# AHartmaier/pyLabFEA

Measured on AMD Instinct MI355X. Metric: integration-point updates/sec (wall-clock per load step in ms_per_step), higher is better.
Workload: dtype f64

## Files before the change

include/plfx.h:

```cpp
#ifndef PLFX_H
#define PLFX_H

#include <stddef.h>
#include <stdint.h>

#ifdef __cplusplus
extern "C" {
#endif

typedef struct plfx_ctx plfx_ctx;

enum {
    PLFX_ELASTIC = 0,
    PLFX_HILL6 = 1,
    PLFX_PRINC3 = 2,
    PLFX_SVC6 = 3,
    PLFX_TRESCA = 4,
    PLFX_BARLAT = 5,
    PLFX_SVC3 = 6,
    PLFX_SVC_WH = 7,
    PLFX_SVC6_COLS = 8
};

enum {
// ... 90 lines not shown
int plfx_set_precond(plfx_ctx *ctx, int kind, double omega, int nu);
int plfx_precond_info(plfx_ctx *ctx, int *kind_in_use, int *levels);
int plfx_precond_apply(plfx_ctx *ctx, const double *r, double *z);
int plfx_precond_bench(plfx_ctx *ctx, int reps, double *us_per_cycle, double *us_coarse);
int plfx_solve_fallbacks(plfx_ctx *ctx, int64_t *count);
int plfx_indefinite_info(plfx_ctx *ctx, int64_t *solves, int64_t *by_minres_surrogate, int64_t *by_gmres,
                         int64_t *surrogates_built, int64_t *elements_shifted);
int plfx_set_operator(plfx_ctx *ctx, int kind);
int plfx_matvec(plfx_ctx *ctx, const double *x, double *y);
int plfx_operator_info(plfx_ctx *ctx, int *matrix_free, int *levels_matrix_free);
int plfx_reuse_info(plfx_ctx *ctx, int *assemblies, int *bc_applications, int *solves);
int plfx_predict_info(plfx_ctx *ctx, int64_t *applied, int64_t *skipped, int64_t *rejected);
int plfx_sweep_info(plfx_ctx *ctx, int64_t *sweeps, int64_t *tangents_rewritten);
int plfx_sweep_launch_info(plfx_ctx *ctx, int64_t *heavy_skipped, int64_t *heavy_recovered);
int plfx_bc_info(plfx_ctx *ctx, int64_t *rhs_rows_only, int64_t *dinv_kept, int64_t *dinv_refreshed, int64_t *du_early);
int plfx_dead_store_info(plfx_ctx *ctx, int64_t *armed_sweeps, int64_t *tangents_rewritten_in_armed_sweeps,
                         int64_t *test_only_starts, int64_t *test_only_retries);
enum {
    PLFX_PLANE_ON = 0,
    PLFX_PLANE_NEVER_ON = 1,
    PLFX_PLANE_SWITCH = 2,
    PLFX_PLANE_SHARDED = 3,
    PLFX_PLANE_MATERIALS = 4,
    PLFX_PLANE_STATE_SET = 5,
    PLFX_PLANE_TANGENT_SET = 6
};
int plfx_plane_info(plfx_ctx *ctx, int *mode_on, int64_t *plane_sweeps, int64_t *plane_updates, int *switched_off_by);
enum {
    PLFX_MG_TAIL_NONE = 0,
    PLFX_MG_TAIL_GENERIC = 1,
// ... 133 lines not shown
```

pylabfea_amd/_lib.py:

```python
import ctypes as C
import os

import numpy as np

_HERE = os.path.dirname(os.path.abspath(__file__))
LIB_PATH = os.environ.get('PLFX_LIB', os.path.join(_HERE, 'libplfx.so'))

ELASTIC, HILL6, PRINC3, SVC6, TRESCA, BARLAT, SVC3, SVC_WH, SVC6_COLS = 0, 1, 2, 3, 4, 5, 6, 7, 8

ST_SIG, ST_EPS, ST_EPL, ST_RES_SIG, ST_RES_DEPL, ST_ELSTIFF, ST_U, ST_F, ST_DU, ST_FYN, ST_MAXSTEPS, ST_KHARD = range(12)

FIELD_NAMES = ('strain1', 'strain2', 'strain12', 'stress1', 'stress2', 'stress12', 'plastic1', 'plastic2', 'plastic12',
               'seq', 'seqJ2', 'peeq', 'etot', 'ux', 'uy')
FIELD_ID = {n: i for i, n in enumerate(FIELD_NAMES)}

T_SWEEP, T_SPMV, T_CGUPD, T_ASSEMBLE, T_VCYCLE, T_SMOOTH, T_SWEEP_HEAVY, T_COMM = range(8)


class PlfxError(RuntimeError):
    pass


class CMaterial(C.Structure):
    _fields_ = [('kind', C.c_int32), ('sdim', C.c_int32), ('CV', C.c_double * 36),
# ... 17 lines not shown
    'plfx_precond_info', 'plfx_set_operator', 'plfx_operator_info', 'plfx_gen_structured', 'plfx_reuse_info', 'plfx_timing_select', 'plfx_finish_fetch', 'plfx_sweep_info', 'plfx_matvec', 'plfx_set_bc_plan', 'plfx_apply_bc_plan',
    'plfx_set_finish_set', 'plfx_finish_step', 'plfx_scf_all', 'plfx_comm_info', 'plfx_comm_init_callback',
    'plfx_set_bc_sources',
    'plfx_load_step', 'plfx_set_strip', 'plfx_strip_info', 'plfx_allreduce_host',
    'plfx_response_batch_kh', 'plfx_fgrad_batch_wh', 'plfx_timing_sample', 'plfx_solve_fallbacks', 'plfx_comm_selftest',
    'plfx_indefinite_info', 'plfx_pattern_selftest', 'plfx_precond_bench', 'plfx_set_wh_mode', 'plfx_wh_info', 'plfx_wh_carry', 'plfx_set_mesh_structured',
    'plfx_svc_info', 'plfx_fgrad_seq_batch', 'plfx_precond_apply', 'plfx_predict_info',
    'plfx_set_response_maxit', 'plfx_sig_princ_host', 'plfx_eig3_host',
    'plfx_svc_fit_batch', 'plfx_svc_decision_batch', 'plfx_svc_fit_wide', 'plfx_hessian_batch',
    'plfx_svr_fit_batch', 'plfx_svr_predict_multi', 'plfx_set_svr_flow', 'plfx_svr_flow_info',
    'plfx_sweep_launch_info', 'plfx_element_fields', 'plfx_bc_info', 'plfx_yield_scale',
    'plfx_committee_yf', 'plfx_committee_info',
    'plfx_tex_svc_set', 'plfx_tex_svc_yf', 'plfx_tex_svc_yield_scale', 'plfx_tex_svc_info',
    'plfx_tex_svc_fgrad', 'plfx_tex_svc_full_yf', 'plfx_tex_svc_response', 'plfx_tex_svc_flow_info',
    'plfx_flow_curve', 'plfx_flow_info',
    'plfx_dead_store_info', 'plfx_plane_info',
    'plfx_set_svc_cols', 'plfx_mg_info',
    'plfx_set_svc_textures', 'plfx_set_element_textures', 'plfx_response_batch_tid', 'plfx_full_yf_batch_tid',
    'plfx_svc_textures_info',
]

_lib = None


def load():
    global _lib
    if _lib is not None:
        return _lib
    if not os.path.exists(LIB_PATH):
        raise PlfxError('libplfx.so not found at %s - build it first (__graft_entry__.build()); '
                        'pylabfea_amd has no CPU fallback' % LIB_PATH)
# ... 609 lines not shown
    def sweep_info(self):
        a, b = C.c_int64(), C.c_int64()
        self._chk(self.lib.plfx_sweep_info(self.h, C.byref(a), C.byref(b)))
        return a.value, b.value

    def sweep_launch_info(self):
        a, b = C.c_int64(), C.c_int64()
        self._chk(self.lib.plfx_sweep_launch_info(self.h, C.byref(a), C.byref(b)))
        return a.value, b.value

    def bc_info(self):
        a, b, r, d = C.c_int64(), C.c_int64(), C.c_int64(), C.c_int64()
        self._chk(self.lib.plfx_bc_info(self.h, C.byref(a), C.byref(b), C.byref(r), C.byref(d)))
        return a.value, b.value, r.value, d.value

    def dead_store_info(self):
        a, b, r, d = C.c_int64(), C.c_int64(), C.c_int64(), C.c_int64()
        self._chk(self.lib.plfx_dead_store_info(self.h, C.byref(a), C.byref(b), C.byref(r), C.byref(d)))
        return a.value, b.value, r.value, d.value

    PLANE_OFF_REASONS = ('on', 'no state reset yet', 'switch', 'sharded', 'materials', 'state_set', 'tangent set')

    def plane_info(self):
        on, a, b, why = C.c_int(), C.c_int64(), C.c_int64(), C.c_int()
        self._chk(self.lib.plfx_plane_info(self.h, C.byref(on), C.byref(a), C.byref(b), C.byref(why)))
        return bool(on.value), a.value, b.value, why.value

    MG_TAIL_KERNELS = ('none', 'tail', 'tail_lds', 'tail_mf', 'tail_mf_ragged')
    MG_COARSE_SOLVERS = ('dense', 'cheby', 'pcg')

# ... 310 lines not shown
```

pylabfea_amd/csrc/plfx.hip:

```cpp
#include "../../include/plfx.h"
#include "plfx_kernels.hpp"
#include "plfx_mg.hpp"
#include "plfx_tex.hpp"
#include "plfx_texflow.hpp"
#include "plfx_flow.hpp"

#include <dlfcn.h>
#include <algorithm>
#include <chrono>
#include <thread>
#include <cmath>
#include <cstdarg>
#include <cstdio>
#include <cstring>
#include <map>
#include <mutex>
#include <string>
#include <type_traits>
#include <vector>

using namespace plfx;

#define PLFX_VERSION "0.1.0-r1"

// ... 190 lines not shown
    std::vector<int32_t> bc_idx;
    bool bc_valid = false;
    double *stage = nullptr;
    size_t stage_cap = 0;
    hipEvent_t stage_ev[2] = {nullptr, nullptr};
    bool stage_busy[2] = {false, false};
    int stage_flip = 0;
    int32_t *bc_idx_dev = nullptr;
    size_t bc_idx_cap = 0;
    int32_t *bc_rows = nullptr;
    int bc_nrows = 0;
    double *kw = nullptr;
    bool bc_rows_on = true;
    bool rhs_rows_ok = false, dinv_ok = false;
    long long n_rhs_rows = 0, n_dinv_kept = 0, n_dinv_refreshed = 0, n_du_early = 0;
    int last_heavy = -1;
    long long n_heavy_skipped = 0, n_heavy_recovered = 0;
    bool x_is_du = false;
    double *pred_x = nullptr, *pred_d = nullptr;
    bool pred_valid = false;
    bool predict = true;
    bool mg_pending = false, mg_pending_same = true;
    long long n_mg_setup = 0, n_mg_setup_skipped = 0;
    bool spec_arm = false, spec_setup = false, spec_kdu = false, spec_was_clean = false;
    bool dead_stores = true, test_starts = true, dead_arm = false, res_partial = false;
    long long n_dead_sweeps = 0, n_dead_tangents = 0, n_test_starts = 0, n_test_retries = 0;
    bool plane_switch = true, plane_mats_ok = false, plane_cols = false;
    int plane_off_by = PLFX_PLANE_NEVER_ON;
    long long n_plane_sweeps = 0, n_plane_updates = 0;
    bool first_test_hint[2] = {false, false};
// ... 574 lines not shown
    dfree(c->f);
    dfree(c->du);
    dfree(c->rhs);
    dfree(c->dinv);
    dfree(c->diag);
    dfree(c->is_presc);
    dfree(c->dup);
    dfree(c->wv);
    dfree(c->fext);
    dfree(c->x);
    dfree(c->r);
    dfree(c->z);
    dfree(c->q);
    dfree(c->pred_x);
    dfree(c->pred_d);
    c->pred_valid = false;
    for (auto &b : c->gm_blk) dfree(b);
    c->gm_blk.clear();
    c->gm_m = 0;
    dfree(c->gm_part);
    dfree(c->gm_part2);
    dfree(c->gm_red);
    dfree(c->gm_coef);
    dfree(c->p[0]);
    dfree(c->p[1]);
    for (auto &L : c->mg) {
        if (!L.owned) continue;
        dfree(L.col);
        dfree(L.contrib);
        dfree(L.cls0);
        dfree(L.val);
// ... 18 lines not shown
    c->val_valid = false;
    c->mg_tail = -1;
    c->gx = c->gy = 0;
    c->assembled = c->bc_set = false;
    c->M_dirty = true;
    c->x_is_du = false;
    c->bc_valid = false;
    c->bc_idx.clear();
    c->plan.valid = false;
    dfree(c->fin_idx);
    dfree(c->fin_dev);
    c->fin_n = 0;
    dfree(c->kw);
    dfree(c->bc_rows);
    c->bc_nrows = 0;
    c->rhs_rows_ok = c->dinv_ok = false;
    dfree(c->tex_ids);
    c->htex_ids.clear();
    c->tex_ids_ok = false;
}

void free_tex_field(plfx_ctx *c, int k)
{
    TexFieldDev &f = c->tex_field[k];
    if (f.coef) hipFree((void *)f.coef);
    if (f.sabs) hipFree((void *)f.sabs);
    f = TexFieldDev();
    c->tex_field_mask &= ~(1u << k);
    c->tex_field_rows[k] = 0;
    c->tex_field_launches[k] = 0;
    c->tex_ids_ok = false;
// ... 254 lines not shown
    KOp o;
    o.rx = rx;
    o.ry = ry;
    o.nnode = nnode;
    o.nslot = nslot;
    o.col = col;
    o.val = val;
    o.nxn = nx + 1;
    o.nyn = ny + 1;
    o.nel = nel;
    o.M = M;
    o.tab = c->dtab;
    return o;
}

int assemble_fine_val(plfx_ctx *c)
{
    hipLaunchKernelGGL(k_assemble, dim3(grid_for(c->nnode), c->nslot), dim3(BLOCK), 0, c->stream,
                       c->dcls, c->ncls, c->nnode, c->nslot, c->nq, c->nel_total, c->dcontrib, c->dcls_all,
                       (matfree(c) && c->assembled) ? c->Mop : c->Mel, c->dcol, c->dval, c->diag,
                       (matfree(c) && c->assembled) ? 1 : 0);
    HIPCHK(c, hipGetLastError());
    c->dinv_ok = false;
    c->val_valid = true;
    return 0;
}

static bool level_plain(const plfx_ctx::MgLevel &L) { return !(L.nx & 1) && !(L.ny & 1) && L.rx == 1. && L.ry == 1.; }

static bool level_from_generators(const plfx_ctx *c, int l)
{
    return matfree(c) && (c->mg[l].matfree || (tail_mf(c) && l < (int)c->mg.size() - 1));
// ... 241 lines not shown
    c->mg_graph = nullptr;
    auto &S = c->strip;
    if (S.x_down) hipGraphExecDestroy(S.x_down);
    if (S.x_up) hipGraphExecDestroy(S.x_up);
    if (S.g_down) hipGraphDestroy(S.g_down);
    if (S.g_up) hipGraphDestroy(S.g_up);
    S.x_down = S.x_up = nullptr;
    S.g_down = S.g_up = nullptr;
}

int mg_assemble(plfx_ctx *c);
int mg_update_dinv(plfx_ctx *c, bool same_set);
bool mg_lazy(const plfx_ctx *c) { return c->predict && matfree(c) && !c->strip.on && !comm_active(c); }
int mg_ensure(plfx_ctx *c)
{
    if (!c->mg_pending) return 0;
    c->mg_pending = false;
    c->n_mg_setup++;
    int rc = mg_assemble(c);
    if (rc) return rc;
    return mg_update_dinv(c, c->mg_pending_same);
}

int mg_vcycle_head(plfx_ctx *c)
{
    if (c->strip_jacobi) return 0;
    const int nl = (int)c->mg.size();
    const int lt = (c->mg_tail > 0) ? c->mg_tail : nl - 1;
    if (lt >= 1) return mg_down_level(c, 0);
    return 0;
}

int mg_vcycle_rest(plfx_ctx *c, double *rz_part, bool *wrote)
{
// ... 180 lines not shown
    HIPCHK(c, hipStreamCreateWithFlags(&c->stream, hipStreamNonBlocking));
    if (const char *e2 = getenv("PLFX_MATFREE")) c->want_matfree = atoi(e2) ? 1 : 0;
    if (const char *e3 = getenv("PLFX_SVC_WAVE")) c->want_svc_wave = atoi(e3) ? 1 : 0;
    if (const char *e4 = getenv("PLFX_COLL_TIMEOUT")) c->coll_timeout_s = atof(e4);
    if (const char *e4 = getenv("PLFX_MG_GRAPH")) c->want_mg_graph = atoi(e4) ? 1 : 0;
    if (const char *e8 = getenv("PLFX_REUSE")) c->reuse = atoi(e8) != 0;
    if (const char *e9 = getenv("PLFX_BC_ROWS")) c->bc_rows_on = atoi(e9) != 0;
    if (const char *e10 = getenv("PLFX_DEAD_STORES")) {
        const int v = atoi(e10);
        c->dead_stores = v == 1 || v == 2;
        c->test_starts = v == 1 || v == 3;
    }
    if (!c->reuse) c->dead_stores = c->test_starts = false;
    if (const char *e11 = getenv("PLFX_PLANE_COLS")) c->plane_switch = atoi(e11) != 0;
    if (!c->reuse) c->plane_switch = false;
    if (const char *e9 = getenv("PLFX_PREDICT")) c->predict = atoi(e9) != 0;
    {
        const char *e5 = getenv("PLFX_MAILBOX");
        if (!e5 || atoi(e5)) {
            if (hipHostMalloc((void **)&c->mbox, sizeof(CgMbox), hipHostMallocMapped | hipHostMallocCoherent) == hipSuccess)
                memset(c->mbox, 0, sizeof(CgMbox));
            else
                c->mbox = nullptr;
            c->mb_cap = 1 << 16;
            if (c->mbox && hipHostMalloc((void **)&c->mb_buf, (size_t)8 * c->mb_cap,
                                         hipHostMallocMapped | hipHostMallocCoherent) != hipSuccess) {
                c->mb_buf = nullptr;
                c->mb_cap = 0;
            }
        }
// ... 1939 lines not shown
    k->grid_nodes = grid_xcd(k->nnode);
    k->op = make_op(k, k->nnode, 0, nullptr, nullptr, k->gx, k->gy, k->nel_total, k->Mop);
    rc = build_hierarchy(k, k->gx, k->gy, c->hcls[0]);
    if (rc || !mg_active(k)) {
        if (!rc) rc = fail(c, PLFX_ERR_UNSUPPORTED, "the global coarse grid %d x %d has no usable hierarchy", k->gx, k->gy);
        else c->err = k->err;
        strip_free(c);
        return rc;
    }
    S.on = true;
    c->grid_nodes = MAXPART;
    c->assembled = false, c->M_dirty = true;
    c->bc_set = false;
    c->bc_valid = false;
    c->rhs_rows_ok = c->dinv_ok = false;
    c->x_is_du = false;
    c->memo.valid = false;
    return PLFX_OK;
}

int plfx_strip_info(plfx_ctx *c, int *active, int *halo, int *coarse_level, int *coarse_levels, int64_t *halo_refreshes,
                    int64_t *coarse_gathers, int64_t *partial_allreduces, int64_t *generator_exchanges)
{
    if (!c) return PLFX_ERR_ARG;
    const auto &S = c->strip;
    if (active) *active = S.on ? 1 : 0;
    if (halo) *halo = S.W;
    if (coarse_level) *coarse_level = S.Ld;
    if (coarse_levels) *coarse_levels = S.child ? (int)S.child->mg.size() : 0;
    if (halo_refreshes) *halo_refreshes = S.n_halo;
// ... 46 lines not shown
int plfx_sweep_info(plfx_ctx *c, int64_t *sweeps, int64_t *tangents_rewritten)
{
    if (!c) return PLFX_ERR_ARG;
    if (sweeps) *sweeps = c->n_sweeps;
    if (tangents_rewritten) *tangents_rewritten = c->n_tangents_rewritten;
    return PLFX_OK;
}

int plfx_bc_info(plfx_ctx *c, int64_t *rhs_rows_only, int64_t *dinv_kept, int64_t *dinv_refreshed, int64_t *du_early)
{
    if (!c) return PLFX_ERR_ARG;
    if (rhs_rows_only) *rhs_rows_only = c->n_rhs_rows;
    if (dinv_kept) *dinv_kept = c->n_dinv_kept;
    if (dinv_refreshed) *dinv_refreshed = c->n_dinv_refreshed;
    if (du_early) *du_early = c->n_du_early;
    return PLFX_OK;
}

int plfx_dead_store_info(plfx_ctx *c, int64_t *armed_sweeps, int64_t *tangents_rewritten_in_armed_sweeps, int64_t *test_only_starts,
                         int64_t *test_only_retries)
{
    if (!c) return PLFX_ERR_ARG;
    if (armed_sweeps) *armed_sweeps = c->n_dead_sweeps;
    if (tangents_rewritten_in_armed_sweeps) *tangents_rewritten_in_armed_sweeps = c->n_dead_tangents;
    if (test_only_starts) *test_only_starts = c->n_test_starts;
    if (test_only_retries) *test_only_retries = c->n_test_retries;
    return PLFX_OK;
}

int plfx_plane_info(plfx_ctx *c, int *mode_on, int64_t *plane_sweeps, int64_t *plane_updates, int *switched_off_by)
// ... 332 lines not shown
        c->kh_out_valid = false;
    }
    hipLaunchKernelGGL(k_init_tangent, dim3((c->nel + BLOCK - 1) / BLOCK), dim3(BLOCK), 0, c->stream,
                       c->dmat, c->dcls, c->nel, c->dcls_id, tan_store(c), c->Mel + c->e0, c->nel_total);
    if (c->sharded)
        hipLaunchKernelGGL(k_init_M_all, dim3((c->nel_total + BLOCK - 1) / BLOCK), dim3(BLOCK), 0, c->stream,
                           c->dmat, c->dcls, c->nel_total, c->dcls_all, c->Mel);
    HIPCHK(c, hipGetLastError());
    c->plane_off_by = !c->plane_switch ? PLFX_PLANE_SWITCH : (c->sharded || c->strip.on || comm_active(c)) ? PLFX_PLANE_SHARDED :
                      !c->plane_mats_ok ? PLFX_PLANE_MATERIALS : PLFX_PLANE_ON;
    c->plane_cols = c->plane_off_by == PLFX_PLANE_ON;
    if (c->plane_cols) HIPCHK(c, hipMemsetAsync(c->elfac + 4 * ne, 0, 16 * ne, c->stream));
    c->assembled = false, c->M_dirty = true;
    c->x_is_du = false;
    c->rhs_rows_ok = c->dinv_ok = false;
    c->res_is_sig = c->res_fresh = c->eps_stale = c->res_partial = false;
    c->last_heavy = -1;
    return PLFX_OK;
}

static int ensure_eps(plfx_ctx *c)
{
    if (!c->eps_stale) return 0;
    hipLaunchKernelGGL(k_eps_from_u, dim3(grid_for(c->nel, MAXPART)), dim3(BLOCK), 0, c->stream, c->dmat, c->nmat, c->dcls, c->ncls,
                       c->nel, c->e0, c->dconn, c->dcls_id, (const double2 *)c->u, c->eps);
    HIPCHK(c, hipGetLastError());
    c->eps_stale = false;
    return 0;
}

// ... 107 lines not shown

int plfx_state_set(plfx_ctx *c, int which, const double *in)
{
    if (!c || !c->sig) return c ? fail(c, PLFX_ERR_STATE, "set_mesh first") : PLFX_ERR_STATE;
    if (!in) return fail(c, PLFX_ERR_ARG, "null input");
    if (which == 10) return fail(c, PLFX_ERR_ARG, "max_steps is read-only");
    double *p;
    size_t comps, n;
    bool soa;
    int rc = (which == 0 || which == 3) ? split_res_sig(c) : 0;
    if (rc) return rc;
    rc = state_ptr(c, which, &p, &comps, &n, &soa);
    if (rc) return rc;
    if (!soa) {
        c->x_is_du = false;
        HIPCHK(c, hipMemcpyAsync(p, in, 8 * n, hipMemcpyHostToDevice, c->stream));
        HIPCHK(c, stream_sync(c));
        return PLFX_OK;
    }
    std::vector<double> t(comps * n);
    if (comps == 6) {
        for (size_t e = 0; e < n; e++)
            for (int k = 0; k < 6; k++) t[(size_t)k * n + e] = in[6 * e + k];
    } else {
        for (size_t e = 0; e < n; e++)
            for (int i = 0; i < 6; i++)
                for (int j = i; j < 6; j++) t[(size_t)sym_idx(i, j) * n + e] = in[36 * e + 6 * i + j];
    }
    if (c->plane_cols && (which == 0 || which == 2 || which == 3 || which == 4)) {
        const double *c34 = t.data() + 3 * n;
// ... 123 lines not shown
    rowptr[2 * nn] = (int32_t)pos;
    return PLFX_OK;
}

namespace {
int apply_bc_impl(plfx_ctx *c, int n, const int32_t *idx, const double *du_presc, const double *w, const double *fext,
                  const int32_t *seg4, const BcSegVals *segv)
{
    const size_t nd = c->ndof;
    int rc = ensure_tmp(c, std::max(n, 1));
    if (rc) return rc;
    const bool same_set = c->bc_valid && (int)c->bc_idx.size() == n &&
                          (n == 0 || memcmp(c->bc_idx.data(), idx, (size_t)4 * n) == 0);
    if (!same_set) {
        c->x_is_du = false;
        HIPCHK(c, hipMemsetAsync(c->is_presc, 0, 8 * nd, c->stream));
        HIPCHK(c, hipMemsetAsync(c->dup, 0, 8 * nd, c->stream));
        HIPCHK(c, hipMemsetAsync(c->wv, 0, 8 * nd, c->stream));
        c->bc_idx.assign(idx, idx + n);
        if ((size_t)n > c->bc_idx_cap) {
            dfree(c->bc_idx_dev);
            if ((rc = dalloc(c, &c->bc_idx_dev, (size_t)n))) return rc;
            c->bc_idx_cap = n;
        }
        if (n > 0) {
            HIPCHK(c, hipMemcpyAsync(c->bc_idx_dev, c->bc_idx.data(), (size_t)4 * n, hipMemcpyHostToDevice, c->stream));
        }
        {
            std::vector<char> mark(c->nnode, 0);
            const int nn = c->nnode;
// ... 68 lines not shown
    {
        if (matfree(c) && c->op.colr)
            hipLaunchKernelGGL(HIP_KERNEL_NAME(k_spmv_rows<2>), dim3((c->bc_nrows + BLOCK - 1) / BLOCK), dim3(BLOCK), 0,
                               c->stream, c->bc_nrows, c->bc_rows, c->op, (const double2 *)c->wv, (double2 *)c->kw, rm, rr);
        else if (matfree(c))
            hipLaunchKernelGGL(HIP_KERNEL_NAME(k_spmv_rows<1>), dim3((c->bc_nrows + BLOCK - 1) / BLOCK), dim3(BLOCK), 0,
                               c->stream, c->bc_nrows, c->bc_rows, c->op, (const double2 *)c->wv, (double2 *)c->kw, rm, rr);
        else
            hipLaunchKernelGGL(HIP_KERNEL_NAME(k_spmv_rows<0>), dim3((c->bc_nrows + BLOCK - 1) / BLOCK), dim3(BLOCK), 0,
                               c->stream, c->bc_nrows, c->bc_rows, c->op, (const double2 *)c->wv, (double2 *)c->kw, rm, rr);
    }
    if (rows_only) {
        c->n_rhs_rows++;
        if (c->dinv_ok)
            c->n_dinv_kept++;
        else {
            hipLaunchKernelGGL(k_dinv, dim3(grid_for(nd)), dim3(BLOCK), 0, c->stream, nd, c->diag, c->is_presc, c->dinv);
            c->n_dinv_refreshed++;
        }
    } else {
        hipLaunchKernelGGL(k_bc_finish, dim3(grid_for(nd)), dim3(BLOCK), 0, c->stream, nd,
                           fext ? c->fext : nullptr, c->kw, c->diag, c->is_presc, c->rhs, c->dinv);
        c->rhs_rows_ok = !fext;
    }
    c->dinv_ok = true;
    HIPCHK(c, hipGetLastError());
    if (fext) HIPCHK(c, stream_sync(c));
    if (mg_active(c)) {
        if (c->mg_pending)
            c->mg_pending_same = c->mg_pending_same && same_set;
        else {
            rc = mg_update_dinv(c, same_set);
            if (rc) return rc;
        }
    }
    if (c->strip.on && (rc = strip_child_dinv(c))) return rc;
    c->bc_set = true;
    return PLFX_OK;
// ... 445 lines not shown
    double *P_rz = c->part + 3 * MAXPART, *P_rr = c->part + 4 * MAXPART, *P_bb = c->part + 5 * MAXPART;
    const bool use_mg = mg_active(c);
    auto apply_B = [&]() -> int {
        int e;
        if (c->strip.on && (e = halo_refresh(c, c->r))) return e;
        if (use_mg) return mg_vcycle(c);
        hipLaunchKernelGGL(k_jacobi_z, dim3(grid_for(nn)), dim3(BLOCK), 0, c->stream, nn, (const double2 *)c->dinv,
                           (const double2 *)c->r, (double2 *)c->z, c->sc);
        return 0;
    };
    int itn = 0, cycles = 0, poor = 0;
    double rl = 0., rr_prev = -1.;
    std::vector<double> H((size_t)(M + 1) * M), cs(M), sn(M), g(M + 1), hcol(M + 2);
    std::vector<double> Hraw((size_t)(M + 1) * M);
    static const bool gm_dbg = getenv("PLFX_GMRES_DEBUG") != nullptr;
    while (true) {
        LAUNCH_OP1(k_cg_start, matfree(c), dim3(gn), c->op, nn, 1, (const double2 *)c->x, (const double2 *)c->rhs,
                   (const double2 *)c->dinv, (double2 *)c->r, (double2 *)c->z, P_rz, P_rr, P_bb, olo, ohi);
        HIPCHK(c, hipGetLastError());
        double o[3];
        if ((rc = host_sums(c, P_rz, 3, gn, o))) return rc;
        const double rr = o[1], bb = o[2];
        hipLaunchKernelGGL(k_cg_setup, dim3(1), dim3(BLOCK), 0, c->stream, P_bb, gn, rtol, c->sc);
        const double tol = rtol * std::sqrt(bb);
        rl = bb > 0. ? std::sqrt(rr / bb) : 0.;
        if (getenv("PLFX_SOLVE_DEBUG")) fprintf(stderr, "[gmres] cycle %d starts at iteration %d: true relative residual %.3e\n", cycles, itn, rl);
        if (rr_prev >= 0. && rr > 0.25 * rr_prev) poor++;
        else poor = 0;
        rr_prev = rr;
        if (std::sqrt(rr) <= tol || itn >= maxit || poor >= 2 || cycles >= 20) {
// ... 142 lines not shown
    }
}

struct SolveRun {
    double *P_pq, *P_rz[2], *P_rr[2], *P_bb;
    int olo, ohi, gn, nn;
    size_t nd;
    bool multi, mg;
    CgScalars hs;
    int done, it;
    bool pred_active, pred_fused;
    bool pred_d_ready, pred_moved;
    bool pred_finished;
    bool du_early;
    bool test_only;
};

bool wait_first_on() { static const bool on = !(getenv("PLFX_WAIT_FIRST") && atoi(getenv("PLFX_WAIT_FIRST")) == 0); return on; }

bool solve_debug_on() { static const bool on = getenv("PLFX_SOLVE_DEBUG") && atoi(getenv("PLFX_SOLVE_DEBUG")) != 0; return on; }

int precondition_rz(plfx_ctx *c, double *slot, EvPair *vcycle_ev = nullptr)
{
    bool fused = false;
    const int rc = mg_vcycle_rest(c, slot, &fused);
    tim_end(c, vcycle_ev);
    if (rc) return rc;
    if (!fused)
        hipLaunchKernelGGL(k_dot_rz, dim3(c->grid_nodes), dim3(BLOCK), 0, c->stream, own_lo(c), own_hi(c), (const double2 *)c->r,
                           (const double2 *)c->z, slot);
// ... 24 lines not shown
{
    int rc;
    if (c->strip.on && (rc = halo_refresh(c, c->x))) return rc;
    hipLaunchKernelGGL(k_compose_du, dim3(grid_for(c->ndof)), dim3(BLOCK), 0, c->stream, c->ndof, c->x, c->dup, c->is_presc, c->du);
    HIPCHK(c, hipGetLastError());
    return 0;
}

void remember(plfx_ctx *c, double rtol, double relres, bool valid) { c->memo = {valid, rtol, relres}; }

int solve_start(plfx_ctx *c, SolveRun &s, double rtol, int warm, int site)
{
    const size_t nd = s.nd;
    const int nn = s.nn, gn = s.gn;
    const bool x_kept = warm && c->x_is_du;
    if (!x_kept)
        hipLaunchKernelGGL(k_x0, dim3(grid_for(nd)), dim3(BLOCK), 0, c->stream, nd, c->du, c->is_presc, warm, 1., c->x);
    c->x_is_du = false;
    int rc = 0;
    const long long nn_global = c->strip.on ? (long long)(c->strip.gnx + 1) * (c->gy + 1) : (long long)c->nnode;
    if (c->predict && warm && !s.multi && mg_active(c) && nn_global >= 16384) {
        if (!c->pred_x && (rc = dalloc(c, &c->pred_x, nd))) return rc;
        if (!c->pred_d && (rc = dalloc(c, &c->pred_d, nd))) return rc;
        if (c->pred_valid)
            s.pred_active = true;
        else {
            HIPCHK(c, hipMemcpyAsync(c->pred_x, c->x, 8 * nd, hipMemcpyDeviceToDevice, c->stream));
            c->pred_valid = true;
        }
    } else
        c->pred_valid = false;
    s.pred_fused = s.pred_active && matfree(c) && !c->op.colr && !c->strip.on && !comm_active(c) && site >= 0 && !c->first_test_hint[site];
    if (s.pred_fused) {
        hipLaunchKernelGGL(k_pred_diff, dim3(grid_for(nd)), dim3(BLOCK), 0, c->stream, nd, c->x, c->pred_x, c->dinv, c->pred_d,
                           (const CgScalars *)nullptr);
        hipLaunchKernelGGL(k_cg_start_pred, dim3(gn), dim3(BLOCK), 0, c->stream, c->op, nn, (const double2 *)c->x, (const double2 *)c->pred_d,
                           (const double2 *)c->rhs, (const double2 *)c->dinv, (double2 *)c->r, (double2 *)c->p[0], s.P_rr[1], s.P_bb);
    } else if (c->test_starts && s.mg && wait_first_on() && s.pred_active && site >= 0 && c->first_test_hint[site] && !c->strip.on &&
               !comm_active(c) && matfree(c)) {
#define TEST_START(G)                                                                                                          \
    hipLaunchKernelGGL(HIP_KERNEL_NAME(k_cg_start_test<G>), dim3(gn), dim3(BLOCK), 0, c->stream, c->op, nn, 1, (const double2 *)c->x, \
                       (const double2 *)c->rhs, (const double2 *)c->dinv, s.P_rr[1], s.P_bb, s.olo, s.ohi)
        if (c->op.colr) TEST_START(2); else TEST_START(1);
#undef TEST_START
        s.test_only = true;
        c->n_test_starts++;
    } else
        LAUNCH_OP1(k_cg_start, matfree(c), dim3(gn), c->op, nn, warm ? 1 : 0, (const double2 *)c->x, (const double2 *)c->rhs,
                   (const double2 *)c->dinv, (double2 *)c->r, (double2 *)c->z, s.P_rz[1], s.P_rr[1], s.P_bb, s.olo, s.ohi);
    if (c->strip.on) {
        if ((rc = part_allreduce(c, s.P_rz[1], (size_t)3 * MAXPART))) return rc;
        if ((rc = halo_refresh(c, c->r))) return rc;
    }
    if (!s.mg) hipLaunchKernelGGL(k_cg_setup, dim3(1), dim3(BLOCK), 0, c->stream, s.P_bb, gn, rtol, c->sc);
    return 0;
}

int solve_first_test(plfx_ctx *c, SolveRun &s, double rtol, int site)
{
    const size_t nd = s.nd;
    const int nn = s.nn, gn = s.gn, olo = s.olo, ohi = s.ohi;
    int rc;
    bool first_passed = false, pred_first_passed = false;
    unsigned long long seq = cg_setup_check_post(c, s.P_bb, s.P_rr[1], gn, rtol);
    const bool wait_first = wait_first_on();
    if (wait_first && s.pred_active && site >= 0 && c->first_test_hint[site] && !c->strip.on) {
        const bool early = c->bc_rows_on && c->reuse && !comm_active(c);
        if (early) {
            hipLaunchKernelGGL(k_compose_du, dim3(grid_for(nd)), dim3(BLOCK), 0, c->stream, nd, c->x, c->dup, c->is_presc, c->du,
                               (const CgScalars *)c->sc);
            HIPCHK(c, hipGetLastError());
        }
        if ((rc = cg_check_wait(c, seq, &s.hs))) return rc;
        s.done = s.hs.done;
        first_passed = s.done != 0;
        if (early && s.done == 1) {
            s.du_early = true;
            c->n_du_early++;
        }
        if (s.test_only && !first_passed) {
            LAUNCH_OP1(k_cg_start, matfree(c), dim3(gn), c->op, nn, 1, (const double2 *)c->x, (const double2 *)c->rhs,
                       (const double2 *)c->dinv, (double2 *)c->r, (double2 *)c->z, s.P_rz[1], s.P_rr[1], s.P_bb, olo, ohi);
            HIPCHK(c, hipGetLastError());
            s.test_only = false;
            c->n_test_retries++;
        }
    }
    if (first_passed) {
        pred_first_passed = true;
    } else if (s.pred_active) {
        if (!s.pred_fused) {
            hipLaunchKernelGGL(k_pred_diff, dim3(grid_for(nd)), dim3(BLOCK), 0, c->stream, nd, c->x, c->pred_x, c->dinv, c->pred_d, c->sc);
            LAUNCH_OP2(k_spmv, 0, matfree(c), dim3(gn), c->op, 0, nn, (const double2 *)c->pred_d, nullptr, nullptr, (double2 *)c->p[0],
                       nullptr, nullptr, nullptr, 0, nullptr, c->sc, 0, 0, 0);
        }
        const int gp = MAXPART;
        hipLaunchKernelGGL(k_pred_dots, dim3(gp), dim3(BLOCK), 0, c->stream, (size_t)2 * olo, (size_t)2 * ohi, c->dinv, c->r, c->p[0],
                           c->part, c->sc);
        HIPCHK(c, hipGetLastError());
        if (c->strip.on && (rc = part_allreduce(c, c->part, (size_t)2 * MAXPART))) return rc;
        hipLaunchKernelGGL(k_pred_try, dim3(gn), dim3(BLOCK), 0, c->stream, nn, c->sc, (const double *)c->part, gp, (const double2 *)c->r,
                           (const double2 *)c->p[0], (const double2 *)c->dinv, s.P_rr[0], olo, ohi);
        HIPCHK(c, hipGetLastError());
        if (c->strip.on && (rc = part_allreduce(c, s.P_rr[0], gn))) return rc;
        seq = cg_check_post(c, s.P_rr[0], gn, -2);
        if (!c->strip.on)
            hipLaunchKernelGGL(k_pred_finish, dim3(grid_for(nd)), dim3(BLOCK), 0, c->stream, nd, (const CgScalars *)c->sc, c->x,
                               (const double *)c->pred_d, c->pred_x, (const double *)c->dup, (const double *)c->is_presc, c->du);
        if ((rc = cg_check_wait(c, seq, &s.hs))) return rc;
        s.done = s.hs.done;
        if (s.done == 1 && s.hs.iters == -2) {
            if (!c->strip.on)
                s.pred_finished = true;
            else
                hipLaunchKernelGGL(k_pred_commit, dim3(grid_for(nd)), dim3(BLOCK), 0, c->stream, nd, (const CgScalars *)c->sc, c->x, c->pred_d);
            HIPCHK(c, hipGetLastError());
            s.hs.iters = 0;
            c->n_pred++;
            s.pred_d_ready = true;
            s.pred_moved = true;
        } else if (!s.done) {
            s.pred_d_ready = true;
            if (s.hs.aux > 0.) c->n_pred_rejected++;
            else c->n_pred_skipped++;
        }
        if (!s.done) {
            if ((rc = mg_ensure(c))) return rc;
            if ((rc = mg_vcycle_head(c))) return rc;
        }
        pred_first_passed = s.done == 1 && !s.pred_moved;
    } else if (c->mg_pending) {
        if ((rc = cg_check_wait(c, seq, &s.hs))) return rc;
        s.done = s.hs.done;
        if (!s.done) {
            if ((rc = mg_ensure(c))) return rc;
            if ((rc = mg_vcycle_head(c))) return rc;
        }
    } else {
        if ((rc = mg_vcycle_head(c))) return rc;
        if ((rc = cg_check_wait(c, seq, &s.hs))) return rc;
        s.done = s.hs.done;
    }
    if (site >= 0 && s.pred_active) c->first_test_hint[site] = pred_first_passed;
    return 0;
}

int pcg_iterate(plfx_ctx *c, SolveRun &s, int maxit)
{
    const int nn = s.nn, gn = s.gn, olo = s.olo, ohi = s.ohi;
    const bool mg = s.mg, multi = s.multi;
    double *const P_pq = s.P_pq, *const *P_rz = s.P_rz, *const *P_rr = s.P_rr;
    CgScalars &hs = s.hs;
    int rc;
    const int chunk = mg ? 1 : 50;
    int &it = s.it;
    while (it < maxit && !s.done) {
        const int stop = std::min(maxit, it + chunk);
        for (; it < stop; it++) {
            const int cur = it & 1;
            const int prev = cur ^ 1;
            double *pold = c->p[prev], *pnew = c->p[cur];
            EvPair *ev;
            tim_begin(c, 1, &ev);
            launch_direction(c, s, it);
            tim_end(c, ev);
            if ((rc = part_allreduce(c, P_pq, gn))) return rc;
            if (multi) {
                hipLaunchKernelGGL(k_p_update_outside, dim3(gn), dim3(BLOCK), 0, c->stream, nn, c->own_n0,
                                   c->own_n1, (const double2 *)pold, (const double2 *)c->z, (double2 *)pnew,
                                   (double2 *)c->q, P_rz[prev], P_rz[cur], P_rr[prev], gn, c->sc);
// ... 103 lines not shown
            }
            fprintf(stderr, "\n      elstiff(21) =");
            for (int k = 0; k < 21; k++) fprintf(stderr, " %.5e", v[k]);
            hipMemcpy(&ms, c->max_steps + e, 4, hipMemcpyDeviceToHost);
            hipMemcpy(&fy, c->fyn + e, 8, hipMemcpyDeviceToHost);
            fprintf(stderr, "\n      max_steps %d  fyn %.6e\n", ms, fy);
        }
    }
}

int finish_by_gmres(plfx_ctx *c, const SolveRun &s, double rtol, int maxit_all, int *iters, double *relres)
{
    int itm = 0, rc;
    double rl = 0.;
    c->n_indefinite++;
    const int rcm = gmres_solve(c, rtol, maxit_all, &itm, &rl);
    if (rcm < 0) return rcm;
    c->n_gmres++;
    if (solve_debug_on()) fprintf(stderr, "[plfx_solve] GMRES(%d): rc %d, %d iterations, relative residual %.3e\n", c->gm_m, rcm, itm, rl);
    if ((rc = compose_du(c))) return rc;
    c->x_is_du = true;
    if (iters) *iters = s.it + itm;
    if (relres) *relres = rl;
    c->pred_valid = false;
    remember(c, rtol, rl, rcm == 0);
    return rcm == 0 ? PLFX_OK : 1;
}

int fall_back_to_jacobi(plfx_ctx *c, const SolveRun &s, double rtol, int maxit_all, int *iters, double *relres)
{
    int rc;
    if ((rc = compose_du(c))) return rc;
    const int saved = c->precond;
    if (c->strip.on) c->strip_jacobi = true;
    else c->precond = 0;
    c->mg_fallbacks++;
    int it2 = 0;
    const int rc2 = solve_impl(c, rtol, maxit_all, 1, -1, &it2, relres);
    if (c->strip.on) c->strip_jacobi = false;
    else c->precond = saved;
    if (!c->strip.on && solve_debug_on()) fprintf(stderr, "[plfx_solve] Jacobi fall-back: rc %d, %d iterations, relative residual %.3e\n", rc2, it2, relres ? *relres : -1.);
    if (iters) *iters = s.it + it2;
    return rc2;
}

int solve_finish(plfx_ctx *c, SolveRun &s, double rtol, int *iters, double *relres)
{
    const size_t nd = s.nd;
    CgScalars &hs = s.hs;
    int rc, done = s.done;
    const int it = s.it;
    if (done == 2) done = 0;
    if (!done) {
        hipLaunchKernelGGL(k_cg_final, dim3(1), dim3(BLOCK), 0, c->stream, s.P_rr[(it - 1) & 1], s.gn, c->sc);
        HIPCHK(c, hipMemcpyAsync(&hs, c->sc, sizeof(hs), hipMemcpyDeviceToHost, c->stream));
        HIPCHK(c, stream_sync(c));
    }
    if (!s.pred_finished && !s.du_early && (rc = compose_du(c))) return rc;
    c->x_is_du = true;
    const int its_done = (done && hs.iters >= 0) ? hs.iters : it;
    if (s.pred_d_ready && !s.pred_finished && (s.pred_moved || its_done > 0))
        hipLaunchKernelGGL(k_pred_advance, dim3(grid_for(nd)), dim3(BLOCK), 0, c->stream, nd, c->pred_x, c->pred_d);
    if (iters) *iters = its_done;
    if (c->tim.on && done) {
        c->tim.noop[1] += it - hs.iters;
        c->tim.noop[2] += it - hs.iters;
    }
    const double bb = hs.thresh2 / (rtol * rtol);
    const double rl = (bb > 0. && hs.rr_final >= 0.) ? std::sqrt(hs.rr_final / bb) : 0.;
    if (relres) *relres = rl;
    remember(c, rtol, rl, done == 1);
    return done ? PLFX_OK : 1;
}

int solve_impl(plfx_ctx *c, double rtol, int maxit, int warm, int site, int *iters, double *relres)
{
    c->spec_setup = c->spec_kdu = false;
// ... 736 lines not shown
```

pylabfea_amd/csrc/plfx_kernels.hpp:

```cpp
#pragma once
#include "plfx_device.hpp"
#include "plfx_rayroot.hpp"

namespace plfx {

constexpr int BLOCK = 256;
constexpr int MAXMAT = 16;
constexpr int MAXCLS = 16;
constexpr int MAXPART = 1024;
#ifndef PLFX_SWEEP_WAVES
#define PLFX_SWEEP_WAVES 1
#endif

struct ClassDev {
    double bxs[4], bys[4];
    double Sxx[16], Sxy[16], Syy[16];
    double kappa, vel, lx, ly;
    int32_t mat, _pad;
};

__device__ __forceinline__ double wave_sum(double v)
{
#pragma unroll
    for (int off = 32; off > 0; off >>= 1) v += __shfl_down(v, off, 64);
// ... 2716 lines not shown
        const double ry = (dv.y != 0.) ? fma(-alpha, ki.y, ri.y) : 0.;
        a_rr = fma(rx, rx, fma(ry, ry, a_rr));
    }
    const double t = block_sum(a_rr, sh);
    if (threadIdx.x == 0) part_rr_out[blockIdx.x] = t;
}

__global__ void __launch_bounds__(BLOCK)
k_pred_commit(size_t ndof, const CgScalars *__restrict__ sc, double *__restrict__ x, const double *__restrict__ d)
{
    const double alpha = sc->aux;
    for (size_t i = blockIdx.x * (size_t)BLOCK + threadIdx.x; i < ndof; i += (size_t)gridDim.x * BLOCK) x[i] = fma(alpha, d[i], x[i]);
}

__global__ void __launch_bounds__(BLOCK)
k_pred_finish(size_t ndof, const CgScalars *__restrict__ sc, double *__restrict__ x, const double *__restrict__ d,
              double *__restrict__ xprev, const double *__restrict__ dup, const double *__restrict__ is_presc, double *__restrict__ du)
{
    if (!(sc->done == 1 && sc->iters == -2)) return;
    const double alpha = sc->aux;
    for (size_t i = blockIdx.x * (size_t)BLOCK + threadIdx.x; i < ndof; i += (size_t)gridDim.x * BLOCK) {
        const double di = d[i];
        const double xi = fma(alpha, di, x[i]);
        x[i] = xi;
        du[i] = (is_presc[i] != 0.) ? dup[i] : xi;
        xprev[i] += di;
    }
}

__global__ void __launch_bounds__(BLOCK)
k_axpy_uf(size_t ndof, const double *__restrict__ du, const double *__restrict__ q, double *__restrict__ u, double *__restrict__ f)
{
    for (size_t i = blockIdx.x * (size_t)BLOCK + threadIdx.x; i < ndof; i += (size_t)gridDim.x * BLOCK) {
        u[i] += du[i];
        f[i] += q[i];
    }
}

template <int SUMS, bool PLANE>
__device__ __forceinline__ void
update_state_body(const MatDev *__restrict__ gmat, int nmat, const ClassDev *__restrict__ gcls, int ncls, int nel, int e_off, const int32_t *__restrict__ conn,
// ... 582 lines not shown
```

Before: 5.304 billion.

## Defer Jacobi diagonal inverse until needed and keep predictor direction across solves

Adds a short-solve mode. When the multigrid setup is still pending, forming the inverse diagonal in BC application is postponed until an operator actually needs it. Separately, k_pred_finish now writes the next predictor difference in place, so the following solve can skip the k_pred_diff launch when x is kept. This removes kernel launches and memory passes on steps that converge at the predictor, at the cost of more invalidation bookkeeping and a risk of using a stale direction or dinv if a path misses an ensure call.

```diff
diff --git a/include/plfx.h b/include/plfx.h
--- a/include/plfx.h
+++ b/include/plfx.h
@@ -128,6 +128,7 @@
 int plfx_sweep_info(plfx_ctx *ctx, int64_t *sweeps, int64_t *tangents_rewritten);
 int plfx_sweep_launch_info(plfx_ctx *ctx, int64_t *heavy_skipped, int64_t *heavy_recovered);
 int plfx_bc_info(plfx_ctx *ctx, int64_t *rhs_rows_only, int64_t *dinv_kept, int64_t *dinv_refreshed, int64_t *du_early);
+int plfx_short_info(plfx_ctx *ctx, int64_t *dinv_deferred, int64_t *dinv_formed_late, int64_t *d_kept, int64_t *spec_merged);
 int plfx_dead_store_info(plfx_ctx *ctx, int64_t *armed_sweeps, int64_t *tangents_rewritten_in_armed_sweeps,
                          int64_t *test_only_starts, int64_t *test_only_retries);
 enum {
diff --git a/pylabfea_amd/_lib.py b/pylabfea_amd/_lib.py
--- a/pylabfea_amd/_lib.py
+++ b/pylabfea_amd/_lib.py
@@ -55,7 +55,7 @@
     'plfx_tex_svc_set', 'plfx_tex_svc_yf', 'plfx_tex_svc_yield_scale', 'plfx_tex_svc_info',
     'plfx_tex_svc_fgrad', 'plfx_tex_svc_full_yf', 'plfx_tex_svc_response', 'plfx_tex_svc_flow_info',
     'plfx_flow_curve', 'plfx_flow_info',
-    'plfx_dead_store_info', 'plfx_plane_info',
+    'plfx_dead_store_info', 'plfx_plane_info', 'plfx_short_info',
     'plfx_set_svc_cols', 'plfx_mg_info',
     'plfx_set_svc_textures', 'plfx_set_element_textures', 'plfx_response_batch_tid', 'plfx_full_yf_batch_tid',
     'plfx_svc_textures_info',
@@ -695,6 +695,11 @@
         self._chk(self.lib.plfx_bc_info(self.h, C.byref(a), C.byref(b), C.byref(r), C.byref(d)))
         return a.value, b.value, r.value, d.value
 
+    def short_info(self):
+        a, b, r, d = C.c_int64(), C.c_int64(), C.c_int64(), C.c_int64()
+        self._chk(self.lib.plfx_short_info(self.h, C.byref(a), C.byref(b), C.byref(r), C.byref(d)))
+        return a.value, b.value, r.value, d.value
+
     def dead_store_info(self):
         a, b, r, d = C.c_int64(), C.c_int64(), C.c_int64(), C.c_int64()
         self._chk(self.lib.plfx_dead_store_info(self.h, C.byref(a), C.byref(b), C.byref(r), C.byref(d)))
diff --git a/pylabfea_amd/csrc/plfx.hip b/pylabfea_amd/csrc/plfx.hip
--- a/pylabfea_amd/csrc/plfx.hip
+++ b/pylabfea_amd/csrc/plfx.hip
@@ -228,6 +228,9 @@
     bool bc_rows_on = true;
     bool rhs_rows_ok = false, dinv_ok = false;
     long long n_rhs_rows = 0, n_dinv_kept = 0, n_dinv_refreshed = 0, n_du_early = 0;
+    int short_solve = 3;
+    bool dinv_late = false, pred_d_kept = false;
+    long long n_dinv_deferred = 0, n_dinv_late = 0, n_d_kept = 0;
     int last_heavy = -1;
     long long n_heavy_skipped = 0, n_heavy_recovered = 0;
     bool x_is_du = false;
@@ -832,7 +835,7 @@
     dfree(c->q);
     dfree(c->pred_x);
     dfree(c->pred_d);
-    c->pred_valid = false;
+    c->pred_valid = c->pred_d_kept = false;
     for (auto &b : c->gm_blk) dfree(b);
     c->gm_blk.clear();
     c->gm_m = 0;
@@ -881,7 +884,7 @@
     dfree(c->kw);
     dfree(c->bc_rows);
     c->bc_nrows = 0;
-    c->rhs_rows_ok = c->dinv_ok = false;
+    c->rhs_rows_ok = c->dinv_ok = c->dinv_late = false;
     dfree(c->tex_ids);
     c->htex_ids.clear();
     c->tex_ids_ok = false;
@@ -1166,8 +1169,19 @@
     return o;
 }
 
+int ensure_dinv(plfx_ctx *c)
+{
+    if (!c->dinv_late) return 0;
+    hipLaunchKernelGGL(k_dinv, dim3(grid_for(c->ndof)), dim3(BLOCK), 0, c->stream, (size_t)c->ndof, c->diag, c->is_presc, c->dinv);
+    HIPCHK(c, hipGetLastError());
+    c->dinv_late = false;
+    c->n_dinv_late++;
+    return 0;
+}
+
 int assemble_fine_val(plfx_ctx *c)
 {
+    if (int rc = ensure_dinv(c)) return rc;
     hipLaunchKernelGGL(k_assemble, dim3(grid_for(c->nnode), c->nslot), dim3(BLOCK), 0, c->stream,
                        c->dcls, c->ncls, c->nnode, c->nslot, c->nq, c->nel_total, c->dcontrib, c->dcls_all,
                        (matfree(c) && c->assembled) ? c->Mop : c->Mel, c->dcol, c->dval, c->diag,
@@ -1439,10 +1453,12 @@
 bool mg_lazy(const plfx_ctx *c) { return c->predict && matfree(c) && !c->strip.on && !comm_active(c); }
 int mg_ensure(plfx_ctx *c)
 {
+    int rc = ensure_dinv(c);
+    if (rc) return rc;
     if (!c->mg_pending) return 0;
     c->mg_pending = false;
     c->n_mg_setup++;
-    int rc = mg_assemble(c);
+    rc = mg_assemble(c);
     if (rc) return rc;
     return mg_update_dinv(c, c->mg_pending_same);
 }
@@ -1653,6 +1669,8 @@
     if (!c->reuse) c->dead_stores = c->test_starts = false;
     if (const char *e11 = getenv("PLFX_PLANE_COLS")) c->plane_switch = atoi(e11) != 0;
     if (!c->reuse) c->plane_switch = false;
+    if (const char *e12 = getenv("PLFX_SHORT_SOLVE")) c->short_solve = atoi(e12) & 3;
+    if (!c->reuse) c->short_solve = 0;
     if (const char *e9 = getenv("PLFX_PREDICT")) c->predict = atoi(e9) != 0;
     {
         const char *e5 = getenv("PLFX_MAILBOX");
@@ -3622,6 +3640,7 @@
     c->bc_set = false;
     c->bc_valid = false;
     c->rhs_rows_ok = c->dinv_ok = false;
+    c->dinv_late = c->pred_d_kept = false;
     c->x_is_du = false;
     c->memo.valid = false;
     return PLFX_OK;
@@ -3698,6 +3717,16 @@
     if (dinv_kept) *dinv_kept = c->n_dinv_kept;
     if (dinv_refreshed) *dinv_refreshed = c->n_dinv_refreshed;
     if (du_early) *du_early = c->n_du_early;
+    return PLFX_OK;
+}
+
+int plfx_short_info(plfx_ctx *c, int64_t *dinv_deferred, int64_t *dinv_formed_late, int64_t *d_kept, int64_t *spec_merged)
+{
+    if (!c) return PLFX_ERR_ARG;
+    if (dinv_deferred) *dinv_deferred = c->n_dinv_deferred;
+    if (dinv_formed_late) *dinv_formed_late = c->n_dinv_late;
+    if (d_kept) *d_kept = c->n_d_kept;
+    if (spec_merged) *spec_merged = 0;
     return PLFX_OK;
 }
 
@@ -4060,6 +4089,7 @@
     c->assembled = false, c->M_dirty = true;
     c->x_is_du = false;
     c->rhs_rows_ok = c->dinv_ok = false;
+    c->pred_d_kept = false;
     c->res_is_sig = c->res_fresh = c->eps_stale = c->res_partial = false;
     c->last_heavy = -1;
     return PLFX_OK;
@@ -4197,6 +4227,7 @@
     if (rc) return rc;
     if (!soa) {
         c->x_is_du = false;
+        c->pred_d_kept = false;
         HIPCHK(c, hipMemcpyAsync(p, in, 8 * n, hipMemcpyHostToDevice, c->stream));
         HIPCHK(c, stream_sync(c));
         return PLFX_OK;
@@ -4350,6 +4381,7 @@
                           (n == 0 || memcmp(c->bc_idx.data(), idx, (size_t)4 * n) == 0);
     if (!same_set) {
         c->x_is_du = false;
+        c->pred_d_kept = false;
         HIPCHK(c, hipMemsetAsync(c->is_presc, 0, 8 * nd, c->stream));
         HIPCHK(c, hipMemsetAsync(c->dup, 0, 8 * nd, c->stream));
         HIPCHK(c, hipMemsetAsync(c->wv, 0, 8 * nd, c->stream));
@@ -4448,14 +4480,20 @@
         c->n_rhs_rows++;
         if (c->dinv_ok)
             c->n_dinv_kept++;
-        else {
+        else if ((c->short_solve & 1) && mg_lazy(c) && mg_active(c) && c->mg_pending) {
+            c->dinv_late = true;
+            c->n_dinv_refreshed++;
+            c->n_dinv_deferred++;
+        } else {
             hipLaunchKernelGGL(k_dinv, dim3(grid_for(nd)), dim3(BLOCK), 0, c->stream, nd, c->diag, c->is_presc, c->dinv);
             c->n_dinv_refreshed++;
+            c->dinv_late = false;
         }
     } else {
         hipLaunchKernelGGL(k_bc_finish, dim3(grid_for(nd)), dim3(BLOCK), 0, c->stream, nd,
                            fext ? c->fext : nullptr, c->kw, c->diag, c->is_presc, c->rhs, c->dinv);
         c->rhs_rows_ok = !fext;
+        c->dinv_late = false;
     }
     c->dinv_ok = true;
     HIPCHK(c, hipGetLastError());
@@ -4931,6 +4969,8 @@
     std::vector<double> H((size_t)(M + 1) * M), cs(M), sn(M), g(M + 1), hcol(M + 2);
     std::vector<double> Hraw((size_t)(M + 1) * M);
     static const bool gm_dbg = getenv("PLFX_GMRES_DEBUG") != nullptr;
+    if ((rc = ensure_dinv(c))) return rc;
+    c->pred_d_kept = false;
     while (true) {
         LAUNCH_OP1(k_cg_start, matfree(c), dim3(gn), c->op, nn, 1, (const double2 *)c->x, (const double2 *)c->rhs,
                    (const double2 *)c->dinv, (double2 *)c->r, (double2 *)c->z, P_rz, P_rr, P_bb, olo, ohi);
@@ -5103,6 +5143,7 @@
     bool pred_finished;
     bool du_early;
     bool test_only;
+    bool d_kept;
 };
 
 bool wait_first_on() { static const bool on = !(getenv("PLFX_WAIT_FIRST") && atoi(getenv("PLFX_WAIT_FIRST")) == 0); return on; }
@@ -5157,8 +5198,10 @@
     const size_t nd = s.nd;
     const int nn = s.nn, gn = s.gn;
     const bool x_kept = warm && c->x_is_du;
-    if (!x_kept)
+    if (!x_kept) {
         hipLaunchKernelGGL(k_x0, dim3(grid_for(nd)), dim3(BLOCK), 0, c->stream, nd, c->du, c->is_presc, warm, 1., c->x);
+        c->pred_d_kept = false;
+    }
     c->x_is_du = false;
     int rc = 0;
     const long long nn_global = c->strip.on ? (long long)(c->strip.gnx + 1) * (c->gy + 1) : (long long)c->nnode;
@@ -5170,13 +5213,18 @@
         else {
             HIPCHK(c, hipMemcpyAsync(c->pred_x, c->x, 8 * nd, hipMemcpyDeviceToDevice, c->stream));
             c->pred_valid = true;
+            c->pred_d_kept = false;
         }
     } else
-        c->pred_valid = false;
+        c->pred_valid = c->pred_d_kept = false;
+    s.d_kept = s.pred_active && c->pred_d_kept && x_kept && (c->short_solve & 2) && !c->strip.on && !comm_active(c);
     s.pred_fused = s.pred_active && matfree(c) && !c->op.colr && !c->strip.on && !comm_active(c) && site >= 0 && !c->first_test_hint[site];
     if (s.pred_fused) {
-        hipLaunchKernelGGL(k_pred_diff, dim3(grid_for(nd)), dim3(BLOCK), 0, c->stream, nd, c->x, c->pred_x, c->dinv, c->pred_d,
-                           (const CgScalars *)nullptr);
+        if (s.d_kept)
+            c->n_d_kept++;
+        else
+            hipLaunchKernelGGL(k_pred_diff, dim3(grid_for(nd)), dim3(BLOCK), 0, c->stream, nd, c->x, c->pred_x, c->dinv, c->pred_d,
+                               (const CgScalars *)nullptr);
         hipLaunchKernelGGL(k_cg_start_pred, dim3(gn), dim3(BLOCK), 0, c->stream, c->op, nn, (const double2 *)c->x, (const double2 *)c->pred_d,
                            (const double2 *)c->rhs, (const double2 *)c->dinv, (double2 *)c->r, (double2 *)c->p[0], s.P_rr[1], s.P_bb);
     } else if (c->test_starts && s.mg && wait_first_on() && s.pred_active && site >= 0 && c->first_test_hint[site] && !c->strip.on &&
@@ -5188,14 +5236,19 @@
 #undef TEST_START
         s.test_only = true;
         c->n_test_starts++;
-    } else
+    } else {
+        if ((rc = ensure_dinv(c))) return rc;
         LAUNCH_OP1(k_cg_start, matfree(c), dim3(gn), c->op, nn, warm ? 1 : 0, (const double2 *)c->x, (const double2 *)c->rhs,
                    (const double2 *)c->dinv, (double2 *)c->r, (double2 *)c->z, s.P_rz[1], s.P_rr[1], s.P_bb, s.olo, s.ohi);
+    }
     if (c->strip.on) {
         if ((rc = part_allreduce(c, s.P_rz[1], (size_t)3 * MAXPART))) return rc;
         if ((rc = halo_refresh(c, c->r))) return rc;
     }
-    if (!s.mg) hipLaunchKernelGGL(k_cg_setup, dim3(1), dim3(BLOCK), 0, c->stream, s.P_bb, gn, rtol, c->sc);
+    if (!s.mg) {
+        if ((rc = ensure_dinv(c))) return rc;
+        hipLaunchKernelGGL(k_cg_setup, dim3(1), dim3(BLOCK), 0, c->stream, s.P_bb, gn, rtol, c->sc);
+    }
     return 0;
 }
 
@@ -5222,6 +5275,7 @@
             c->n_du_early++;
         }
         if (s.test_only && !first_passed) {
+            if ((rc = ensure_dinv(c))) return rc;
             LAUNCH_OP1(k_cg_start, matfree(c), dim3(gn), c->op, nn, 1, (const double2 *)c->x, (const double2 *)c->rhs,
                        (const double2 *)c->dinv, (double2 *)c->r, (double2 *)c->z, s.P_rz[1], s.P_rr[1], s.P_bb, olo, ohi);
             HIPCHK(c, hipGetLastError());
@@ -5233,7 +5287,10 @@
         pred_first_passed = true;
     } else if (s.pred_active) {
         if (!s.pred_fused) {
-            hipLaunchKernelGGL(k_pred_diff, dim3(grid_for(nd)), dim3(BLOCK), 0, c->stream, nd, c->x, c->pred_x, c->dinv, c->pred_d, c->sc);
+            if (s.d_kept)
+                c->n_d_kept++;
+            else
+                hipLaunchKernelGGL(k_pred_diff, dim3(grid_for(nd)), dim3(BLOCK), 0, c->stream, nd, c->x, c->pred_x, c->dinv, c->pred_d, c->sc);
             LAUNCH_OP2(k_spmv, 0, matfree(c), dim3(gn), c->op, 0, nn, (const double2 *)c->pred_d, nullptr, nullptr, (double2 *)c->p[0],
                        nullptr, nullptr, nullptr, 0, nullptr, c->sc, 0, 0, 0);
         }
@@ -5249,10 +5306,12 @@
         seq = cg_check_post(c, s.P_rr[0], gn, -2);
         if (!c->strip.on)
             hipLaunchKernelGGL(k_pred_finish, dim3(grid_for(nd)), dim3(BLOCK), 0, c->stream, nd, (const CgScalars *)c->sc, c->x,
-                               (const double *)c->pred_d, c->pred_x, (const double *)c->dup, (const double *)c->is_presc, c->du);
+                               c->pred_d, c->pred_x, (const double *)c->dup, (const double *)c->is_presc, c->du,
+                               ((c->short_solve & 2) && !comm_active(c)) ? 1 : 0);
         if ((rc = cg_check_wait(c, seq, &s.hs))) return rc;
         s.done = s.hs.done;
         if (s.done == 1 && s.hs.iters == -2) {
+            c->pred_d_kept = !c->strip.on && (c->short_solve & 2) && !comm_active(c);
             if (!c->strip.on)
                 s.pred_finished = true;
             else
@@ -5280,6 +5339,7 @@
             if ((rc = mg_vcycle_head(c))) return rc;
         }
     } else {
+        if ((rc = ensure_dinv(c))) return rc;
         if ((rc = mg_vcycle_head(c))) return rc;
         if ((rc = cg_check_wait(c, seq, &s.hs))) return rc;
         s.done = s.hs.done;
@@ -5297,6 +5357,7 @@
     int rc;
     const int chunk = mg ? 1 : 50;
     int &it = s.it;
+    if (it < maxit && !s.done) c->pred_d_kept = false;
     while (it < maxit && !s.done) {
         const int stop = std::min(maxit, it + chunk);
         for (; it < stop; it++) {
@@ -5430,6 +5491,7 @@
     int itm = 0, rc;
     double rl = 0.;
     c->n_indefinite++;
+    c->pred_d_kept = false;
     const int rcm = gmres_solve(c, rtol, maxit_all, &itm, &rl);
     if (rcm < 0) return rcm;
     c->n_gmres++;
@@ -5438,7 +5500,7 @@
     c->x_is_du = true;
     if (iters) *iters = s.it + itm;
     if (relres) *relres = rl;
-    c->pred_valid = false;
+    c->pred_valid = c->pred_d_kept = false;
     remember(c, rtol, rl, rcm == 0);
     return rcm == 0 ? PLFX_OK : 1;
 }
@@ -5446,6 +5508,8 @@
 int fall_back_to_jacobi(plfx_ctx *c, const SolveRun &s, double rtol, int maxit_all, int *iters, double *relres)
 {
     int rc;
+    c->pred_d_kept = false;
+    if ((rc = ensure_dinv(c))) return rc;
     if ((rc = compose_du(c))) return rc;
     const int saved = c->precond;
     if (c->strip.on) c->strip_jacobi = true;
@@ -5475,8 +5539,10 @@
     if (!s.pred_finished && !s.du_early && (rc = compose_du(c))) return rc;
     c->x_is_du = true;
     const int its_done = (done && hs.iters >= 0) ? hs.iters : it;
-    if (s.pred_d_ready && !s.pred_finished && (s.pred_moved || its_done > 0))
+    if (s.pred_d_ready && !s.pred_finished && (s.pred_moved || its_done > 0)) {
         hipLaunchKernelGGL(k_pred_advance, dim3(grid_for(nd)), dim3(BLOCK), 0, c->stream, nd, c->pred_x, c->pred_d);
+        c->pred_d_kept = false;
+    }
     if (iters) *iters = its_done;
     if (c->tim.on && done) {
         c->tim.noop[1] += it - hs.iters;
diff --git a/pylabfea_amd/csrc/plfx_kernels.hpp b/pylabfea_amd/csrc/plfx_kernels.hpp
--- a/pylabfea_amd/csrc/plfx_kernels.hpp
+++ b/pylabfea_amd/csrc/plfx_kernels.hpp
@@ -2754,17 +2754,21 @@
 }
 
 __global__ void __launch_bounds__(BLOCK)
-k_pred_finish(size_t ndof, const CgScalars *__restrict__ sc, double *__restrict__ x, const double *__restrict__ d,
-              double *__restrict__ xprev, const double *__restrict__ dup, const double *__restrict__ is_presc, double *__restrict__ du)
+k_pred_finish(size_t ndof, const CgScalars *__restrict__ sc, double *__restrict__ x, double *__restrict__ d,
+              double *__restrict__ xprev, const double *__restrict__ dup, const double *__restrict__ is_presc, double *__restrict__ du,
+              int keep_d)
 {
     if (!(sc->done == 1 && sc->iters == -2)) return;
     const double alpha = sc->aux;
     for (size_t i = blockIdx.x * (size_t)BLOCK + threadIdx.x; i < ndof; i += (size_t)gridDim.x * BLOCK) {
         const double di = d[i];
         const double xi = fma(alpha, di, x[i]);
+        const double mi = is_presc[i];
         x[i] = xi;
-        du[i] = (is_presc[i] != 0.) ? dup[i] : xi;
-        xprev[i] += di;
+        du[i] = (mi != 0.) ? dup[i] : xi;
+        const double xp = xprev[i] + di;
+        xprev[i] = xp;
+        if (keep_d) d[i] = (mi == 0.) ? xi - xp : 0.;
     }
 }
 
```

Measured after the change: 5.600 billion (median of 6 runs). 5.6% higher.
